# rikace/GameOfLifeWithActors

Measured on AMD Instinct MI355X. Metric: cell updates/sec (GCUPS), whole job over all GPUs, 65536^2 cells per GPU; % of HBM peak BW, higher is better.
Workload: dtype u32 (bit-packed cells); 1 GPU; 65536x65536 torus board, 85312 generations timed in passes of 32 (temporal block), 1 row strip(s); width=65536, height=65536, interleave=4, boundary=torus, seed=24301, parallelism=row strips x1

## Files before the change

gameoflifewithactors_amd/csrc/gol_pipe.hip:

```cpp
#include <hip/hip_runtime.h>
#include <stdint.h>

#include <atomic>
#include <vector>

#include "gol_bitlogic.h"
#include "gol_internal.h"

#define GOL_PIPE_STR2(x) #x
#define GOL_PIPE_STR(x) GOL_PIPE_STR2(x)

namespace gol {

namespace {

constexpr int kWave = 64;
constexpr int kInterior = kWave - 2;
constexpr int kM = 4;
constexpr int kR = 4;
constexpr int kNT = 2;
constexpr int kNoStore = 0x7ffffff0;
constexpr int kRsrcWord3 = 0x00020000;
constexpr int kWaitVm0 = 0x0F70;
constexpr int kAllButDs = 0x1 | 0x2 | 0x4 | 0x8 | 0x10 | 0x20 | 0x40 | 0x400;

typedef uint32_t u32x4 __attribute__((ext_vector_type(4)));

template <bool Z>
__device__ __forceinline__ uint32_t from_left(uint32_t v) {
    return (uint32_t)__builtin_amdgcn_mov_dpp((int)v, Z ? 0x138 : 0x13C, 0xf, 0xf, Z);
}
template <bool Z>
__device__ __forceinline__ uint32_t from_right(uint32_t v) {
    return (uint32_t)__builtin_amdgcn_mov_dpp((int)v, Z ? 0x130 : 0x134, 0xf, 0xf, Z);
}
__device__ __forceinline__ __amdgpu_buffer_rsrc_t rsrc(const void* p, int64_t bytes) {
    return __builtin_amdgcn_make_buffer_rsrc(const_cast<void*>(p), (short)0, (int)bytes, kRsrcWord3);
}
__device__ __forceinline__ uint32_t lds_addr(const void* p) {
    return (uint32_t)(uintptr_t)(const __attribute__((address_space(3))) void*)p;
}
__device__ __forceinline__ void lds_publish(int* p, int v) {
    asm volatile("ds_write_b32 %0, %1" : : "v"(lds_addr(p)), "v"(v) : "memory");
}
#ifndef GOL_PIPE_SLEEP
#define GOL_PIPE_SLEEP 1
#endif
#ifndef GOL_PIPE_POLL_ALIGN
#define GOL_PIPE_POLL_ALIGN 6
#endif
__device__ __forceinline__ int lds_wait(const int* p, int need, int limit) {
    int left = limit, tmp;
    asm volatile(
        "s_branch 2f\n"
        ".p2align " GOL_PIPE_STR(GOL_PIPE_POLL_ALIGN) "\n"
        "1:\n\t"
        "s_sleep " GOL_PIPE_STR(GOL_PIPE_SLEEP) "\n\t"
        "s_sub_i32 %[left], %[left], 1\n\t"
        "s_cmp_le_i32 %[left], 0\n\t"
        "s_cbranch_scc1 3f\n"
        "2:\n\t"
        "ds_read_b32 %[tmp], %[addr]\n\t"
        "s_waitcnt lgkmcnt(0)\n\t"
        "v_cmp_gt_i32 vcc, %[need], %[tmp]\n\t"
        "s_cbranch_vccnz 1b\n"
        "3:"
        : [left] "+s"(left), [tmp] "=&v"(tmp)
        : [addr] "v"(lds_addr(p)), [need] "s"(need)
        : "vcc", "scc", "memory");
    return left;
}
__device__ __forceinline__ void lds_read_trip(const uint32_t* p, u32x4& r0, u32x4& r1, u32x4& r2, u32x4& r3) {
    asm volatile(
        "ds_read_b128 %0, %4\n\tds_read_b128 %1, %4 offset:1024\n\tds_read_b128 %2, %4 offset:2048\n\t"
        "ds_read_b128 %3, %4 offset:3072\n\ts_waitcnt lgkmcnt(0)"
        : "=&v"(r0), "=&v"(r1), "=&v"(r2), "=&v"(r3)
        : "v"(lds_addr(p))
        : "memory");
}
__device__ __forceinline__ void lds_write_row(uint32_t* p, const u32x4& w) {
    asm volatile("ds_write_b128 %0, %1" : : "v"(lds_addr(p)), "v"(w) : "memory");
}

__device__ __forceinline__ int64_t uniform64(int64_t v) {
    const uint64_t u = (uint64_t)v;
    const uint32_t lo = (uint32_t)__builtin_amdgcn_readfirstlane((int)(uint32_t)u);
    const uint32_t hi = (uint32_t)__builtin_amdgcn_readfirstlane((int)(uint32_t)(u >> 32));
    return (int64_t)(((uint64_t)hi << 32) | lo);
}

__host__ __device__ __forceinline__ int64_t pipe_cut(int64_t len, int i, int n, int split1, int split2, int K) {
    if (i <= 0) return 0;
    if (i >= n) return len;
    if (split1 <= 0) return len * i / n;
    const float f1 = (float)split1 * (1.0f / 65536.0f), f2 = (float)(split2 > 0 ? split2 : split1) * (1.0f / 65536.0f);
    const float r1 = (1.0f - f1) / f1, r2 = (1.0f - f2) / f2;
    float pw = 1.0f, sum = 0.0f, head = 0.0f;
    for (int j = 0; j < n; j++) {
        if (j == i) head = sum;
        sum += pw;
        pw *= j == 0 ? r1 : r2;
    }
    const float total = (float)(len + 2 * K * n);
    const int64_t c = (int64_t)(total * head / sum + 0.5f) - 2 * K * i;
    return c < 0 ? 0 : (c > len ? len : c);
}

}

__host__ __device__ __forceinline__ bool pipe_unit(const PipeArgs& a, int64_t grp, int64_t* sx, int64_t* gy, int* cnt) {
    *cnt = 0;
    if (grp < a.nstrips * a.ngroups) {
        *sx = grp % a.nstrips;
        *gy = grp / a.nstrips;
        return true;
    }
    const int64_t r = grp - a.nstrips * a.ngroups;
    if (r >= a.nrem) return false;
    *sx = a.nstrips;
    if (r < a.npk) {
        *gy = a.pk_lo + r * a.rp;
        const int64_t left = a.pk_hi - *gy;
        *cnt = (int)(left < a.rp ? left : a.rp);
    } else {
        const int64_t l = r - a.npk;
        *gy = l < a.pk_lo ? l : a.pk_hi + (l - a.pk_lo);
        *cnt = 1;
    }
    return *gy < a.ngroups;
}

__host__ __device__ __forceinline__ void pipe_rows(const PipeArgs& a, int64_t gy, int p, int K, int64_t* y0, int64_t* L) {
    const int64_t total = a.out_end - a.out_begin;
    const int64_t g0 = gy * a.grows;
    const int64_t glen = a.grows < total - g0 ? a.grows : total - g0;
    const int64_t c0 = pipe_cut(glen, p, a.P, a.split1, a.split2, K), c1 = pipe_cut(glen, p + 1, a.P, a.split1, a.split2, K);
    *y0 = a.out_begin + g0 + c0;
    *L = glen > 0 ? c1 - c0 : 0;
}

template <int D, int S, int P, bool WRAP, bool BND>
__global__ __launch_bounds__(kWave * S * P) __attribute__((amdgpu_waves_per_eu(S * P / 4)))
void gol_pipe_step(const uint32_t* __restrict__ src, uint32_t* __restrict__ dst, PipeArgs a) {
    constexpr int K = D * S, NR = kNT * kR;
    __shared__ __attribute__((aligned(16))) uint32_t dstage[P][2][kR][kWave * kM];
    __shared__ __attribute__((aligned(16))) uint32_t ring[P][S - 1][NR][kWave * kM];
    __shared__ int ctr[P][S][2];
    const int lane = threadIdx.x & (kWave - 1);
    const int wave = __builtin_amdgcn_readfirstlane(threadIdx.x >> 6);
#if defined(GOL_PIPE_MAP) && GOL_PIPE_MAP == 1
    const int p = wave / S, s = S - 1 - (wave % S + p) % S;
#else
    const int p = wave / S, s = (wave % S + p) % S;
#endif
    if (lane == 0) {
        ctr[p][s][0] = 0;
        ctr[p][s][1] = 0;
    }
    __syncthreads();
#if defined(GOL_PIPE_PRIO) && GOL_PIPE_PRIO > 0
    if (GOL_PIPE_PRIO == 1 || GOL_PIPE_PRIO == 4 ? s >= S / 2 : (GOL_PIPE_PRIO == 2 ? s < S / 2 : s == S - 1))
        __builtin_amdgcn_s_setprio(GOL_PIPE_PRIO == 4 ? 0 : 1);
#endif
#ifdef GOL_PIPE_PAD
    asm volatile(".rept " GOL_PIPE_STR(GOL_PIPE_PAD) "\n\ts_nop 0\n\t.endr");
#endif
    int64_t sx, gy;
    int cnt;
    int64_t y0, L;
    if (!pipe_unit(a, blockIdx.x, &sx, &gy, &cnt)) return;
    pipe_rows(a, gy, p, K, &y0, &L);
    y0 = uniform64(y0);
    L = uniform64(L);
    if (L <= 0) return;
    const int n_in = (int)(L + 2 * K - 2 * s * D);
    const int n_out = n_in - 2 * D;
    const int T = (n_in + kR - 1) / kR;
    const int64_t pitch_bytes = a.pitch * 4;
    int64_t cb, delta = 0;
    bool stores;
    if (BND && cnt == 0) {
        const int64_t last = a.nblocks - kWave;
        const int64_t c = sx + 1 < a.nstrips && sx * kInterior < last ? sx * kInterior : last;
        cb = c + lane;
        stores = (c == 0 || lane >= 1) && (c == last || lane <= kInterior);
    } else if (cnt == 0) {
        const int64_t first = sx * kInterior < a.nblocks - kInterior ? sx * kInterior : a.nblocks - kInterior;
        cb = first - 1 + lane;
        stores = lane >= 1 && lane <= kInterior;
    } else {
        const int j = lane / a.rq, i = lane - j * a.rq;
        cb = a.nstrips * kInterior - (BND ? kInterior - 1 : 0) - 1 + i;
        stores = j < cnt && i >= 1 && i <= a.rem;
        delta = j < cnt ? (int64_t)j * a.grows * pitch_bytes : 0;
    }
    cb = cb < 0 ? cb + a.nblocks : (cb >= a.nblocks ? cb - a.nblocks : cb);
    const int load_off = (int)(cb * 4 * kM + delta);
    const int store_off = stores ? load_off : kNoStore;
    const int64_t span = (cnt > 1 ? (int64_t)(cnt - 1) * a.grows * pitch_bytes : 0) + a.words * 4;
    const int64_t buf_rows = WRAP ? a.rows : a.rows + 2 * a.ghost;

    uint32_t sX[D][kM], cX[D][kM], sY[D][kM], cY[D][kM], aY[D][kM];
#pragma unroll
    for (int g = 0; g < D; g++)
#pragma unroll
        for (int j = 0; j < kM; j++) sX[g][j] = cX[g][j] = sY[g][j] = cY[g][j] = aY[g][j] = 0;

    int64_t lrow;
    if (WRAP) {
        lrow = (y0 - K) % a.rows;
        lrow = lrow < 0 ? lrow + a.rows : lrow;
    } else {
        lrow = a.ghost + y0 - K;
    }
    [[maybe_unused]] const int live_blo = (int)a.ghost + a.live_lo, live_bhi = (int)a.ghost + a.live_hi;
    auto dma_trip = [&](int par) {
#pragma unroll
        for (int r = 0; r < kR; r++) {
            int64_t br = lrow;
            bool dead = false;
            if (WRAP) {
                lrow = lrow + 1 == a.rows ? 0 : lrow + 1;
            } else {
                lrow++;
                const int b32 = (int)br, n32 = (int)buf_rows;
                br = b32 < 0 ? 0 : (b32 < n32 ? b32 : n32 - 1);
                dead = BND && (b32 < live_blo || b32 >= live_bhi);
            }
            auto* q = (__attribute__((address_space(3))) void*)&dstage[p][par][r][0];
            __builtin_amdgcn_raw_ptr_buffer_load_lds(rsrc(src + br * a.pitch, dead ? 0 : span), q, 16, load_off, 0, 0, 0);
        }
    };
    bool failed = false;
    const int spin_limit = (int)a.spin_limit;
    auto wait_ge = [&](const int* c, int need) {
        if (lds_wait(c, need, spin_limit) <= 0) {
            if (lane == 0) __hip_atomic_fetch_or(a.err, 2, __ATOMIC_RELAXED, __HIP_MEMORY_SCOPE_AGENT);
            failed = true;
        }
    };

    uint32_t v[kR][kM];
    if (s == 0) dma_trip(0);
    for (int t = 0; t < T && !failed; t++) {
        const int par = t & 1;
        if (s == 0) {
            __builtin_amdgcn_s_waitcnt(kWaitVm0);
#pragma unroll
            for (int r = 0; r < kR; r++) {
                const u32x4 x = *(const u32x4*)&dstage[p][par][r][lane * kM];
                v[r][0] = x.x;
                v[r][1] = x.y;
                v[r][2] = x.z;
                v[r][3] = x.w;
            }
            __builtin_amdgcn_sched_barrier(0);
            if (t + 1 < T) dma_trip(par ^ 1);
        } else {
            lds_publish(&ctr[p][s][1], kR * t);
            wait_ge(&ctr[p][s - 1][0], kR * t + kR < n_in ? kR * t + kR : n_in);
            u32x4 x[kR];
            lds_read_trip(&ring[p][s - 1][(kR * t) % NR][lane * kM], x[0], x[1], x[2], x[3]);
#pragma unroll
            for (int r = 0; r < kR; r++) {
                v[r][0] = x[r].x;
                v[r][1] = x[r].y;
                v[r][2] = x[r].z;
                v[r][3] = x[r].w;
            }
        }
        __builtin_amdgcn_sched_barrier(0);
        [[maybe_unused]] const int yt = (int)(y0 - K + s * D) + kR * t;
        [[maybe_unused]] const bool edge_trip = BND && (yt - D < a.live_lo || yt + kR - 2 >= a.live_hi);
        uint32_t right[kR];
#pragma unroll
        for (int r = 0; r < kR; r++) right[r] = from_right<BND>(v[r][0]);
#pragma unroll
        for (int g = 0; g < D; g++) {
#pragma unroll
            for (int r = 0; r < kR; r += 2) {
                uint32_t o0[kM], o1[kM], sN[kM], cN[kM];
                row_sum_block<kM>(v[r], from_left<BND>(v[r][kM - 1]), right[r], sN, cN);
#pragma unroll
                for (int j = 0; j < kM; j++) {
                    o0[j] = life_next(sX[g][j], cX[g][j], sY[g][j], cY[g][j], sN[j], cN[j], aY[g][j]);
                    sX[g][j] = sN[j];
                    cX[g][j] = cN[j];
                }
                row_sum_block<kM>(v[r + 1], from_left<BND>(v[r + 1][kM - 1]), right[r + 1], sN, cN);
#pragma unroll
                for (int j = 0; j < kM; j++) {
                    o1[j] = life_next(sY[g][j], cY[g][j], sX[g][j], cX[g][j], sN[j], cN[j], v[r][j]);
                    sY[g][j] = sN[j];
                    cY[g][j] = cN[j];
                }
                if constexpr (BND) {
                    if (edge_trip) {
                        const int ya = yt + r - g - 1;
                        const bool da = ya < a.live_lo || ya >= a.live_hi, db = ya + 1 < a.live_lo || ya + 1 >= a.live_hi;
#pragma unroll
                        for (int j = 0; j < kM; j++) {
                            o0[j] = da ? 0u : o0[j];
                            o1[j] = db ? 0u : o1[j];
                        }
                    }
                }
#pragma unroll
                for (int j = 0; j < kM; j++) {
                    aY[g][j] = v[r + 1][j];
                    v[r][j] = o0[j];
                    v[r + 1][j] = o1[j];
                }
                if (g + 1 < D) {
                    right[r] = from_right<BND>(o0[0]);
                    right[r + 1] = from_right<BND>(o1[0]);
                    __builtin_amdgcn_sched_barrier(kAllButDs);
                }
            }
            __builtin_amdgcn_sched_barrier(0);
        }
        const int j0 = kR * t - 2 * D;
        if (s == S - 1) {
#pragma unroll
            for (int r = 0; r < kR; r++) {
                const int j = j0 + r;
                const bool valid = j >= 0 && j < n_out;
                const int64_t y = y0 + (valid ? j : 0);
                const u32x4 w = {v[r][0], v[r][1], v[r][2], v[r][3]};
                __builtin_amdgcn_raw_buffer_store_b128(w, rsrc(dst + ((WRAP ? 0 : a.ghost) + y) * a.pitch, valid ? span : 0),
                                                       store_off, 0, 0);
            }
        } else if (j0 + kR > 0) {
            const int jmax = j0 + kR - 1 < n_out - 1 ? j0 + kR - 1 : n_out - 1;
            wait_ge(&ctr[p][s + 1][1], jmax + 1 - NR);
#pragma unroll
            for (int r = 0; r < kR; r++) {
                const int j = j0 + r;
                if (j >= 0 && j < n_out) lds_write_row(&ring[p][s][j % NR][lane * kM], u32x4{v[r][0], v[r][1], v[r][2], v[r][3]});
            }
            lds_publish(&ctr[p][s][0], j0 + kR < n_out ? j0 + kR : n_out);
        }
    }
}

namespace {

template <int K>
struct PipeShape;
template <>
struct PipeShape<16> {
    static constexpr int D = 4, S = 4, P = 4;
};
template <>
struct PipeShape<32> {
    static constexpr int D = 4, S = 8, P = 2;
};

template <int K>
const void* pipe_kernel(bool wrap, bool bounded) {
    using Sh = PipeShape<K>;
    if (wrap) return (const void*)&gol_pipe_step<Sh::D, Sh::S, Sh::P, true, false>;
    return bounded ? (const void*)&gol_pipe_step<Sh::D, Sh::S, Sh::P, false, true>
                   : (const void*)&gol_pipe_step<Sh::D, Sh::S, Sh::P, false, false>;
}
const void* pipe_kernel_for(int k, bool wrap, bool bounded) {
    if (k == 16) return pipe_kernel<16>(wrap, bounded);
    if (k == 32) return pipe_kernel<32>(wrap, bounded);
    return nullptr;
}
int pipe_pipelines(int k) { return k == 32 ? PipeShape<32>::P : PipeShape<16>::P; }

int64_t pipe_resident_wgs(int k, bool wrap, bool bounded) {
    static std::atomic<int64_t> cache[2][3];
    const int ki = k == 32 ? 1 : 0, vi = wrap ? 0 : (bounded ? 2 : 1);
    int64_t v = cache[ki][vi].load(std::memory_order_relaxed);
    if (v > 0) return v;
    const void* fn = pipe_kernel_for(k, wrap, bounded);
    int dev = 0, cus = 0, blocks = 0;
    if (!fn || hipGetDevice(&dev) != hipSuccess ||
        hipDeviceGetAttribute(&cus, hipDeviceAttributeMultiprocessorCount, dev) != hipSuccess ||
        hipOccupancyMaxActiveBlocksPerMultiprocessor(&blocks, fn, kWave * 16, 0) != hipSuccess || blocks <= 0 || cus <= 0) {
        (void)hipGetLastError();
        return 256;
    }
    v = (int64_t)blocks * cus;
    cache[ki][vi].store(v, std::memory_order_relaxed);
    return v;
}

}

bool pipe_supported(int k) { return k == 16 || k == 32; }

namespace {
__device__ int g_pipe_err;
}

int* pipe_error_word() {
    static int* p = nullptr;
    if (!p) {
        void* q = nullptr;
        if (hipGetSymbolAddress(&q, HIP_SYMBOL(g_pipe_err)) != hipSuccess) {
            (void)hipGetLastError();
            return nullptr;
        }
        p = static_cast<int*>(q);
    }
    return p;
}

bool pipe_applies(int64_t words, int ilv, int k, bool bounded, int rag_bits) {
    return !rag_bits && ilv == kM && pipe_supported(k) && words / kM >= (bounded ? kWave : kInterior);
}

int pipe_default_split(int k) {
    return k == 32 ? (int)(0.75 * 65536) : (int)(0.60 * 65536);
}

void plan_pipe(PipeArgs& a, int k, bool wrap, int64_t spare_waves) {
    a.P = pipe_pipelines(k);
    a.nblocks = a.words / kM;
    a.nstrips = a.nblocks / kInterior;
    a.rem = (int32_t)(a.nblocks - a.nstrips * kInterior);
    a.rq = a.rem + 2;
    a.rp = a.rem ? kWave / a.rq : 0;
    if (a.bounded) {
        const int64_t edge2 = 2 * kWave - 2;
        a.nstrips = a.nblocks <= kWave ? 1 : (a.nblocks < edge2 ? 2 : 2 + (a.nblocks - edge2) / kInterior);
        a.rem = a.nstrips < 2 ? 0 : (int32_t)(a.nblocks - edge2 - (a.nstrips - 2) * kInterior);
        if (a.rem < 0) a.rem = 0;
        a.rq = a.rem + 2;
        a.rp = a.rem ? kWave / a.rq : 0;
    }
    if (a.rem && a.rp < 2) {
        a.nstrips++;
        a.rem = 0;
        a.rq = 2;
        a.rp = 0;
    }
    if (a.split1 == 0) a.split1 = pipe_default_split(k);
    if (a.split1 < 0) a.split1 = 0;
    const int64_t rows = a.out_end - a.out_begin;
    a.ngroups = a.grows = a.npk = a.nrem = 0;
    a.pk_lo = a.pk_hi = 0;
    if (rows <= 0) return;
    int64_t wgs = a.wgs_opt > 0 ? a.wgs_opt : pipe_resident_wgs(k, wrap, a.bounded != 0);
    const int64_t spare = (spare_waves + 15) / 16;
    wgs = wgs > spare + 1 ? wgs - spare : 1;
    const int64_t pitch_bytes = a.pitch * 4;
    const int64_t lo_lim = wrap ? 0 : -a.ghost, hi_lim = wrap ? a.rows : a.rows + a.ghost;
    auto fill = [&](int64_t ng) {
        a.grows = (rows + ng - 1) / ng;
        a.ngroups = (rows + a.grows - 1) / a.grows;
        a.pk_lo = a.pk_hi = a.ngroups;
        a.npk = 0;
        if (a.rem) {
            int rp = a.rp;
            const int64_t fit = 1 + ((((int64_t)1 << 31) - 1 - a.words * 4) / (a.grows * pitch_bytes));
            if (rp > fit) rp = (int)(fit > 1 ? fit : 1);
            a.rp = rp;
            int64_t hi = a.ngroups - 1;
            const int64_t by_rows = (hi_lim - a.out_begin - k - kR) / a.grows;
            if (by_rows < hi) hi = by_rows;
            const bool low_ok = a.out_begin + a.grows - k >= lo_lim;
            if (rp >= 2 && low_ok && hi > 1 && a.grows >= k) {
                a.pk_lo = 1;
                a.pk_hi = hi;
                a.npk = (a.pk_hi - a.pk_lo + rp - 1) / rp;
            }
            a.nrem = a.npk + (a.ngroups - (a.pk_hi - a.pk_lo));
        } else {
            a.nrem = 0;
        }
    };
    int64_t ng = wgs / a.nstrips;
    const int64_t max_ng = rows / (2 * k) > 1 ? rows / (2 * k) : 1;
    if (ng > max_ng) ng = max_ng;
    if (ng < 1) ng = 1;
    for (; ng > 1; ng--) {
        fill(ng);
        if (a.nstrips * a.ngroups + a.nrem <= wgs) break;
    }
    if (ng <= 1) fill(1);
}

int64_t pipe_grid(const PipeArgs& a) { return a.nstrips * a.ngroups + a.nrem; }

int64_t pipe_check_plan(const PipeArgs& a, int k, bool wrap) {
    int64_t bad = 0;
    const int64_t rows = a.out_end - a.out_begin;
    if (rows <= 0) return 0;
    const int64_t pitch_bytes = a.pitch * 4;
    const int64_t lo_lim = wrap ? 0 : -a.ghost, hi_lim = wrap ? a.rows : a.rows + a.ghost;
    std::vector<uint8_t> seen((size_t)(rows * a.nblocks), 0);
    for (int64_t grp = 0; grp < pipe_grid(a); grp++) {
        int64_t sx, gy;
        int cnt;
        if (!pipe_unit(a, grp, &sx, &gy, &cnt)) {
            bad++;
            continue;
        }
        for (int p = 0; p < a.P; p++) {
            int64_t y0, L;
            pipe_rows(a, gy, p, k, &y0, &L);
            if (L <= 0) continue;
            const int64_t n_in = L + 2 * k, streamed = (n_in + kR - 1) / kR * kR;
            for (int lane = 0; lane < kWave; lane++) {
                int64_t cb, delta_rows = 0;
                bool stores;
                if (a.bounded && cnt == 0) {
                    const int64_t last = a.nblocks - kWave;
                    const int64_t c = sx + 1 < a.nstrips && sx * kInterior < last ? sx * kInterior : last;
                    cb = c + lane;
                    stores = (c == 0 || lane >= 1) && (c == last || lane <= kInterior);
                } else if (cnt == 0) {
                    const int64_t first = sx * kInterior < a.nblocks - kInterior ? sx * kInterior : a.nblocks - kInterior;
                    cb = first - 1 + lane;
                    stores = lane >= 1 && lane <= kInterior;
                } else {
                    const int j = lane / a.rq, i = lane - j * a.rq;
                    cb = a.nstrips * kInterior - (a.bounded ? kInterior - 1 : 0) - 1 + i;
                    stores = j < cnt && i >= 1 && i <= a.rem;
                    delta_rows = j < cnt ? (int64_t)j * a.grows : 0;
                    if (j < cnt && (int64_t)j * a.grows * pitch_bytes + a.nblocks * 4 * kM > (((int64_t)1 << 31) - 1)) bad++;
                    if (cnt > 1 && j < cnt) {
                        const int64_t first_row = y0 - k + delta_rows, last_row = y0 - k + streamed - 1 + delta_rows;
                        if (first_row < lo_lim || last_row >= hi_lim) bad++;
                        if ((gy + j + 1) * a.grows > rows) bad++;
                    }
                }
                cb = cb < 0 ? cb + a.nblocks : (cb >= a.nblocks ? cb - a.nblocks : cb);
                if (!stores) continue;
                for (int64_t y = y0 + delta_rows; y < y0 + delta_rows + L; y++) {
                    const int64_t r = y - a.out_begin;
                    if (r < 0 || r >= rows) {
                        bad++;
                        break;
                    }
                    seen[(size_t)(r * a.nblocks + cb)] = 1;
                }
            }
        }
    }
    for (uint8_t s : seen)
        if (!s) bad++;
    return bad;
}

hipError_t launch_pipe_step(const uint32_t* src, uint32_t* dst, PipeArgs a, int k, bool wrap, hipStream_t s) {
    plan_pipe(a, k, wrap, a.spare_waves);
    const int64_t grid = pipe_grid(a);
    if (grid <= 0) return hipSuccess;
    if (!a.err) return hipErrorInvalidValue;
    if (!wrap && a.rows + 2 * a.ghost >= ((int64_t)1 << 31)) return hipErrorInvalidValue;
    if (a.bounded && (wrap || a.nblocks < kWave)) return hipErrorInvalidValue;
    if (a.spin_limit <= 0) a.spin_limit = (int64_t)1 << 22;
    const dim3 block(kWave * 16);
    if (k == 16) {
        using Sh = PipeShape<16>;
        if (wrap)
            hipLaunchKernelGGL((gol_pipe_step<Sh::D, Sh::S, Sh::P, true, false>), dim3((unsigned)grid), block, 0, s, src, dst, a);
        else if (a.bounded)
            hipLaunchKernelGGL((gol_pipe_step<Sh::D, Sh::S, Sh::P, false, true>), dim3((unsigned)grid), block, 0, s, src, dst, a);
        else
            hipLaunchKernelGGL((gol_pipe_step<Sh::D, Sh::S, Sh::P, false, false>), dim3((unsigned)grid), block, 0, s, src, dst, a);
    } else if (k == 32) {
        using Sh = PipeShape<32>;
        if (wrap)
            hipLaunchKernelGGL((gol_pipe_step<Sh::D, Sh::S, Sh::P, true, false>), dim3((unsigned)grid), block, 0, s, src, dst, a);
        else if (a.bounded)
            hipLaunchKernelGGL((gol_pipe_step<Sh::D, Sh::S, Sh::P, false, true>), dim3((unsigned)grid), block, 0, s, src, dst, a);
        else
            hipLaunchKernelGGL((gol_pipe_step<Sh::D, Sh::S, Sh::P, false, false>), dim3((unsigned)grid), block, 0, s, src, dst, a);
    } else {
        return hipErrorInvalidValue;
    }
    return hipGetLastError();
}

}
```

Measured before the change: 149,700 GCUPS.

## Specialize pipeline trips into fill/full/last and precompute LDS addresses

Splits the per-wave trip loop into fill, steady-state and last-trip instantiations so the steady state drops per-row validity checks and bounds clamps. LDS ring and counter addresses become base registers with immediate offsets, using a ring aligned so a toggling XOR selects the half. Source and destination row pointers are advanced incrementally instead of being recomputed from row indices. A failed wait now ends the program directly instead of setting a flag, and padding nops align each generation level. The aim is to cut scalar and vector address arithmetic in the inner pipeline, at the cost of more code, tighter alignment assumptions and an abrupt exit on timeout.

```diff
diff --git a/gameoflifewithactors_amd/csrc/gol_pipe.hip b/gameoflifewithactors_amd/csrc/gol_pipe.hip
--- a/gameoflifewithactors_amd/csrc/gol_pipe.hip
+++ b/gameoflifewithactors_amd/csrc/gol_pipe.hip
@@ -2,6 +2,7 @@
 #include <stdint.h>
 
 #include <atomic>
+#include <type_traits>
 #include <vector>
 
 #include "gol_bitlogic.h"
@@ -19,6 +20,7 @@
 constexpr int kM = 4;
 constexpr int kR = 4;
 constexpr int kNT = 2;
+constexpr int kFillTrip = 0, kFullTrip = 1, kLastTrip = 2;
 constexpr int kNoStore = 0x7ffffff0;
 constexpr int kRsrcWord3 = 0x00020000;
 constexpr int kWaitVm0 = 0x0F70;
@@ -40,8 +42,9 @@
 __device__ __forceinline__ uint32_t lds_addr(const void* p) {
     return (uint32_t)(uintptr_t)(const __attribute__((address_space(3))) void*)p;
 }
-__device__ __forceinline__ void lds_publish(int* p, int v) {
-    asm volatile("ds_write_b32 %0, %1" : : "v"(lds_addr(p)), "v"(v) : "memory");
+template <int OFF>
+__device__ __forceinline__ void lds_publish(uint32_t base, int v) {
+    asm volatile("ds_write_b32 %0, %1 offset:%2" : : "v"(base), "v"(v), "i"(OFF) : "memory");
 }
 #ifndef GOL_PIPE_SLEEP
 #define GOL_PIPE_SLEEP 1
@@ -49,7 +52,8 @@
 #ifndef GOL_PIPE_POLL_ALIGN
 #define GOL_PIPE_POLL_ALIGN 6
 #endif
-__device__ __forceinline__ int lds_wait(const int* p, int need, int limit) {
+template <int OFF>
+__device__ __forceinline__ int lds_wait(uint32_t base, int need, int limit) {
     int left = limit, tmp;
     asm volatile(
         "s_branch 2f\n"
@@ -60,26 +64,34 @@
         "s_cmp_le_i32 %[left], 0\n\t"
         "s_cbranch_scc1 3f\n"
         "2:\n\t"
-        "ds_read_b32 %[tmp], %[addr]\n\t"
+        "ds_read_b32 %[tmp], %[addr] offset:%[off]\n\t"
         "s_waitcnt lgkmcnt(0)\n\t"
         "v_cmp_gt_i32 vcc, %[need], %[tmp]\n\t"
         "s_cbranch_vccnz 1b\n"
         "3:"
         : [left] "+s"(left), [tmp] "=&v"(tmp)
-        : [addr] "v"(lds_addr(p)), [need] "s"(need)
+        : [addr] "v"(base), [need] "s"(need), [off] "i"(OFF)
         : "vcc", "scc", "memory");
     return left;
 }
-__device__ __forceinline__ void lds_read_trip(const uint32_t* p, u32x4& r0, u32x4& r1, u32x4& r2, u32x4& r3) {
+constexpr int kRowBytes = kWave * kM * 4;
+__device__ __forceinline__ void lds_read_trip(uint32_t base, u32x4& r0, u32x4& r1, u32x4& r2, u32x4& r3) {
     asm volatile(
-        "ds_read_b128 %0, %4\n\tds_read_b128 %1, %4 offset:1024\n\tds_read_b128 %2, %4 offset:2048\n\t"
-        "ds_read_b128 %3, %4 offset:3072\n\ts_waitcnt lgkmcnt(0)"
+        "ds_read_b128 %0, %4\n\tds_read_b128 %1, %4 offset:%5\n\tds_read_b128 %2, %4 offset:%6\n\t"
+        "ds_read_b128 %3, %4 offset:%7\n\ts_waitcnt lgkmcnt(0)"
         : "=&v"(r0), "=&v"(r1), "=&v"(r2), "=&v"(r3)
-        : "v"(lds_addr(p))
+        : "v"(base), "i"(kRowBytes), "i"(2 * kRowBytes), "i"(3 * kRowBytes)
         : "memory");
 }
-__device__ __forceinline__ void lds_write_row(uint32_t* p, const u32x4& w) {
-    asm volatile("ds_write_b128 %0, %1" : : "v"(lds_addr(p)), "v"(w) : "memory");
+#ifndef GOL_PIPE_LEVEL_PAD
+#define GOL_PIPE_LEVEL_PAD 1
+#endif
+__device__ __forceinline__ void level_align() {
+    asm volatile(".p2align 3\n\t.rept " GOL_PIPE_STR(GOL_PIPE_LEVEL_PAD) "\n\ts_nop 0\n\t.endr");
+}
+template <int OFF>
+__device__ __forceinline__ void lds_write_row(uint32_t base, const u32x4& w) {
+    asm volatile("ds_write_b128 %0, %1 offset:%2" : : "v"(base), "v"(w), "i"(OFF) : "memory");
 }
 
 __device__ __forceinline__ int64_t uniform64(int64_t v) {
@@ -143,8 +155,9 @@
 __global__ __launch_bounds__(kWave * S * P) __attribute__((amdgpu_waves_per_eu(S * P / 4)))
 void gol_pipe_step(const uint32_t* __restrict__ src, uint32_t* __restrict__ dst, PipeArgs a) {
     constexpr int K = D * S, NR = kNT * kR;
-    __shared__ __attribute__((aligned(16))) uint32_t dstage[P][2][kR][kWave * kM];
-    __shared__ __attribute__((aligned(16))) uint32_t ring[P][S - 1][NR][kWave * kM];
+    __shared__ __attribute__((aligned(2 * kR * kRowBytes))) uint32_t dstage[P][2][kR][kWave * kM];
+    __shared__ __attribute__((aligned(2 * kR * kRowBytes))) uint32_t ring[P][S - 1][NR][kWave * kM];
+    static_assert(kNT == 2 && 2 * D % kR == 0, "a ring of two trips; the fill ends on a trip boundary");
     __shared__ int ctr[P][S][2];
     const int lane = threadIdx.x & (kWave - 1);
     const int wave = __builtin_amdgcn_readfirstlane(threadIdx.x >> 6);
@@ -195,8 +208,10 @@
         delta = j < cnt ? (int64_t)j * a.grows * pitch_bytes : 0;
     }
     cb = cb < 0 ? cb + a.nblocks : (cb >= a.nblocks ? cb - a.nblocks : cb);
+    const uint32_t cbase = lds_addr(&ctr[p][s > 0 ? s - 1 : 0][0]);
     const int load_off = (int)(cb * 4 * kM + delta);
-    const int store_off = stores ? load_off : kNoStore;
+    int aux = s == 0 ? load_off : (s == S - 1 ? (stores ? load_off : kNoStore) : (int)cbase);
+    asm volatile("" : "+v"(aux));
     const int64_t span = (cnt > 1 ? (int64_t)(cnt - 1) * a.grows * pitch_bytes : 0) + a.words * 4;
     const int64_t buf_rows = WRAP ? a.rows : a.rows + 2 * a.ghost;
 
@@ -213,68 +228,79 @@
     } else {
         lrow = a.ghost + y0 - K;
     }
+    const uint32_t* lptr = src + (WRAP ? lrow : (lrow < 0 ? 0 : (lrow < buf_rows ? lrow : buf_rows - 1))) * a.pitch;
     [[maybe_unused]] const int live_blo = (int)a.ghost + a.live_lo, live_bhi = (int)a.ghost + a.live_hi;
     auto dma_trip = [&](int par) {
 #pragma unroll
         for (int r = 0; r < kR; r++) {
-            int64_t br = lrow;
+            const uint32_t* row = lptr;
             bool dead = false;
             if (WRAP) {
-                lrow = lrow + 1 == a.rows ? 0 : lrow + 1;
+                const bool last = lrow + 1 == a.rows;
+                lrow = last ? 0 : lrow + 1;
+                lptr = last ? src : lptr + a.pitch;
             } else {
+                const int b32 = (int)lrow, n32 = (int)buf_rows;
                 lrow++;
-                const int b32 = (int)br, n32 = (int)buf_rows;
-                br = b32 < 0 ? 0 : (b32 < n32 ? b32 : n32 - 1);
+                lptr = b32 >= 0 && b32 < n32 - 1 ? lptr + a.pitch : lptr;
                 dead = BND && (b32 < live_blo || b32 >= live_bhi);
             }
             auto* q = (__attribute__((address_space(3))) void*)&dstage[p][par][r][0];
-            __builtin_amdgcn_raw_ptr_buffer_load_lds(rsrc(src + br * a.pitch, dead ? 0 : span), q, 16, load_off, 0, 0, 0);
+            __builtin_amdgcn_raw_ptr_buffer_load_lds(rsrc(row, dead ? 0 : span), q, 16, aux, 0, 0, 0);
         }
     };
-    bool failed = false;
     const int spin_limit = (int)a.spin_limit;
-    auto wait_ge = [&](const int* c, int need) {
-        if (lds_wait(c, need, spin_limit) <= 0) {
+    constexpr int kCtr = 2 * (int)sizeof(int);
+    constexpr int kFirstOut = 0, kFirstFree = kCtr + 4;
+    constexpr int kPrevOut = 0, kOut = kCtr, kIn = kCtr + 4, kNextFree = 2 * kCtr + 4;
+    auto wait_ge = [&](auto off, uint32_t cb, int need) __attribute__((always_inline)) {
+        if (lds_wait<decltype(off)::value>(cb, need, spin_limit) <= 0) {
             if (lane == 0) __hip_atomic_fetch_or(a.err, 2, __ATOMIC_RELAXED, __HIP_MEMORY_SCOPE_AGENT);
-            failed = true;
+            asm volatile("s_endpgm");
         }
     };
-
-    uint32_t v[kR][kM];
-    if (s == 0) dma_trip(0);
-    for (int t = 0; t < T && !failed; t++) {
-        const int par = t & 1;
+    uint32_t rd = s == 0 ? lds_addr(&dstage[p][0][0][lane * kM]) : lds_addr(&ring[p][s > 0 ? s - 1 : 0][0][lane * kM]);
+    const uint32_t first_ring = lds_addr(&ring[p][0][0][0]) - lds_addr(&dstage[p][0][0][0]);
+    constexpr int kRingBytes = NR * kRowBytes, kHalf = kR * kRowBytes;
+    static_assert(2 * D == NR, "rows out share the parity of rows in");
+    uint32_t* sptr = dst + ((WRAP ? 0 : a.ghost) + y0) * a.pitch;
+
+    auto trip = [&](auto kind, const int t) __attribute__((always_inline)) {
+        constexpr bool FILL = decltype(kind)::value == kFillTrip, FULL = decltype(kind)::value != kLastTrip;
+        const int t4 = kR * t;
+        u32x4 x[kR];
+        const auto ring_in = [&](uint32_t cb) __attribute__((always_inline)) {
+            lds_publish<kIn>(cb, t4);
+            wait_ge(std::integral_constant<int, kPrevOut>{}, cb, FULL || t4 + kR < n_in ? t4 + kR : n_in);
+            lds_read_trip(rd, x[0], x[1], x[2], x[3]);
+        };
         if (s == 0) {
             __builtin_amdgcn_s_waitcnt(kWaitVm0);
-#pragma unroll
-            for (int r = 0; r < kR; r++) {
-                const u32x4 x = *(const u32x4*)&dstage[p][par][r][lane * kM];
-                v[r][0] = x.x;
-                v[r][1] = x.y;
-                v[r][2] = x.z;
-                v[r][3] = x.w;
-            }
+            lds_read_trip(rd, x[0], x[1], x[2], x[3]);
             __builtin_amdgcn_sched_barrier(0);
-            if (t + 1 < T) dma_trip(par ^ 1);
+            if (FULL || t + 1 < T) dma_trip((t & 1) ^ 1);
+        } else if (s == S - 1) {
+            ring_in(cbase);
         } else {
-            lds_publish(&ctr[p][s][1], kR * t);
-            wait_ge(&ctr[p][s - 1][0], kR * t + kR < n_in ? kR * t + kR : n_in);
-            u32x4 x[kR];
-            lds_read_trip(&ring[p][s - 1][(kR * t) % NR][lane * kM], x[0], x[1], x[2], x[3]);
-#pragma unroll
-            for (int r = 0; r < kR; r++) {
-                v[r][0] = x[r].x;
-                v[r][1] = x[r].y;
-                v[r][2] = x[r].z;
-                v[r][3] = x[r].w;
-            }
+            ring_in((uint32_t)aux);
+        }
+        uint32_t v[kR][kM];
+#pragma unroll
+        for (int r = 0; r < kR; r++) {
+            v[r][0] = x[r].x;
+            v[r][1] = x[r].y;
+            v[r][2] = x[r].z;
+            v[r][3] = x[r].w;
         }
         __builtin_amdgcn_sched_barrier(0);
-        [[maybe_unused]] const int yt = (int)(y0 - K + s * D) + kR * t;
+        [[maybe_unused]] const int yt = (int)(y0 - K + s * D) + t4;
         [[maybe_unused]] const bool edge_trip = BND && (yt - D < a.live_lo || yt + kR - 2 >= a.live_hi);
         uint32_t right[kR];
 #pragma unroll
         for (int r = 0; r < kR; r++) right[r] = from_right<BND>(v[r][0]);
+        __builtin_amdgcn_sched_barrier(0);
+        level_align();
+        __builtin_amdgcn_sched_barrier(0);
 #pragma unroll
         for (int g = 0; g < D; g++) {
 #pragma unroll
@@ -318,29 +344,47 @@
                 }
             }
             __builtin_amdgcn_sched_barrier(0);
-        }
-        const int j0 = kR * t - 2 * D;
-        if (s == S - 1) {
+            level_align();
+            __builtin_amdgcn_sched_barrier(0);
+        }
+        const int j0 = t4 - 2 * D;
+        const auto out = [&](int r) __attribute__((always_inline)) { return u32x4{v[r][0], v[r][1], v[r][2], v[r][3]}; };
+        if (FILL) {
+        } else if (s == S - 1) {
 #pragma unroll
             for (int r = 0; r < kR; r++) {
-                const int j = j0 + r;
-                const bool valid = j >= 0 && j < n_out;
-                const int64_t y = y0 + (valid ? j : 0);
-                const u32x4 w = {v[r][0], v[r][1], v[r][2], v[r][3]};
-                __builtin_amdgcn_raw_buffer_store_b128(w, rsrc(dst + ((WRAP ? 0 : a.ghost) + y) * a.pitch, valid ? span : 0),
-                                                       store_off, 0, 0);
+                const bool valid = FULL || (j0 + r >= 0 && j0 + r < n_out);
+                __builtin_amdgcn_raw_buffer_store_b128(out(r), rsrc(sptr, valid ? span : 0), aux, 0, 0);
+                sptr = valid ? sptr + a.pitch : sptr;
             }
-        } else if (j0 + kR > 0) {
-            const int jmax = j0 + kR - 1 < n_out - 1 ? j0 + kR - 1 : n_out - 1;
-            wait_ge(&ctr[p][s + 1][1], jmax + 1 - NR);
-#pragma unroll
-            for (int r = 0; r < kR; r++) {
-                const int j = j0 + r;
-                if (j >= 0 && j < n_out) lds_write_row(&ring[p][s][j % NR][lane * kM], u32x4{v[r][0], v[r][1], v[r][2], v[r][3]});
+        } else if (FULL || j0 + kR > 0) {
+            const int jmax = FULL || j0 + kR - 1 < n_out - 1 ? j0 + kR - 1 : n_out - 1;
+            if (s == 0) {
+                const uint32_t wr0 = rd + first_ring;
+                wait_ge(std::integral_constant<int, kFirstFree>{}, cbase, jmax + 1 - NR);
+                if (FULL || (j0 + 0 >= 0 && j0 + 0 < n_out)) lds_write_row<0 * kRowBytes>(wr0, out(0));
+                if (FULL || (j0 + 1 >= 0 && j0 + 1 < n_out)) lds_write_row<1 * kRowBytes>(wr0, out(1));
+                if (FULL || (j0 + 2 >= 0 && j0 + 2 < n_out)) lds_write_row<2 * kRowBytes>(wr0, out(2));
+                if (FULL || (j0 + 3 >= 0 && j0 + 3 < n_out)) lds_write_row<3 * kRowBytes>(wr0, out(3));
+                lds_publish<kFirstOut>(cbase, jmax + 1);
+            } else {
+                wait_ge(std::integral_constant<int, kNextFree>{}, (uint32_t)aux, jmax + 1 - NR);
+                if (FULL || (j0 + 0 >= 0 && j0 + 0 < n_out)) lds_write_row<kRingBytes + 0 * kRowBytes>(rd, out(0));
+                if (FULL || (j0 + 1 >= 0 && j0 + 1 < n_out)) lds_write_row<kRingBytes + 1 * kRowBytes>(rd, out(1));
+                if (FULL || (j0 + 2 >= 0 && j0 + 2 < n_out)) lds_write_row<kRingBytes + 2 * kRowBytes>(rd, out(2));
+                if (FULL || (j0 + 3 >= 0 && j0 + 3 < n_out)) lds_write_row<kRingBytes + 3 * kRowBytes>(rd, out(3));
+                lds_publish<kOut>((uint32_t)aux, jmax + 1);
             }
-            lds_publish(&ctr[p][s][0], j0 + kR < n_out ? j0 + kR : n_out);
-        }
-    }
+        }
+        rd ^= kHalf;
+    };
+
+    if (s == 0) dma_trip(0);
+    constexpr int kFill = 2 * D / kR;
+    int t = 0;
+    for (; t < kFill; t++) trip(std::integral_constant<int, kFillTrip>{}, t);
+    for (; t < T - 1; t++) trip(std::integral_constant<int, kFullTrip>{}, t);
+    for (; t < T; t++) trip(std::integral_constant<int, kLastTrip>{}, t);
 }
 
 namespace {
```

Measured after the change: 155,000 GCUPS (median of 6 runs). +3.5%, better.
